# Unrepentant-Atheist/AC-3-ACM-Codec

Hardware: AMD Instinct MI355X
Metric: AC-3 5.1@48kHz frames/sec/GPU (decode+encode); achieved HBM GB/s vs peak (higher is better)
Workload: dtype f32+i32

## Files before the change

### ac-3-acm-codec_amd/csrc/enc_syntax.h

```cpp
#pragma once
#include <stdint.h>

#ifndef __HIPCC__
#ifndef __host__
#define __host__
#endif
#ifndef __device__
#define __device__
#endif
#endif

namespace ac3mi {

#define SYN_FN __host__ __device__ inline __attribute__((always_inline))

constexpr int sdecaycod = 2, fdecaycod = 1, sgaincod = 1, dbkneecod = 2, floorcod = 4, fgaincod = 4;
constexpr int CPL_FLEAK = 0, CPL_SLEAK = 0;
constexpr int SYN_CPL = -1;

template <class D>
struct SynWriter {
    uint32_t pos = 0;
    uint64_t acc = 0;
    int nacc = 0;
    SYN_FN void put(int n, uint32_t v) { acc = (acc << n) | v; nacc += n; }
    SYN_FN void flush()
    {
        if (nacc > 32) {
            static_cast<D *>(this)->store(pos, nacc - 32, (uint32_t)(acc >> 32) & (0xffffffffu >> (64 - nacc)));
            pos += nacc - 32;
            nacc = 32;
        }
        if (nacc > 0) {
            static_cast<D *>(this)->store(pos, nacc, (uint32_t)acc & (0xffffffffu >> (32 - nacc)));
            pos += nacc;
            nacc = 0;
        }
    }
};

struct SynCounter {
    int bits = 0;
    SYN_FN void put(int n, uint32_t) { bits += n; }
    SYN_FN void flush() {}
    SYN_FN void exponents(int, int, int ng) { bits += 4 + 7 * ng; }
};

template <class K>
SYN_FN void syn_header(K &k, uint32_t fscod, uint32_t frmsizecod, uint32_t bsid, int acmod, bool lfe, bool dual, uint32_t m,
                       uint32_t compr0, uint32_t compr1)
{
    k.put(16, 0x0b77); k.put(16, 0); k.put(2, fscod); k.put(6, frmsizecod); k.put(5, bsid); k.put(3, (m >> 5) & 7u); k.put(3, (uint32_t)acmod);
    k.flush();
    if ((acmod & 1) && acmod != 1) k.put(2, (m >> 8) & 3u);
    if (acmod & 4) k.put(2, (m >> 10) & 3u);
    if (acmod == 2) k.put(2, (m >> 12) & 3u);
    k.put(1, lfe);
    auto programme = [&](uint32_t c) {
        k.put(5, m & 31u);
        if (c & 0x100u) { k.put(1, 1); k.put(8, c & 0xffu); } else k.put(1, 0);
        k.put(2, 0);
    };
    programme(compr0);
    if (dual) programme(compr1);
    k.put(1, (m >> 14) & 1u); k.put(1, (m >> 15) & 1u); k.put(3, 0);
    k.flush();
}

struct SynShape {
    int acmod, nfbw, nch;
    bool lfe, dual;
    int nbc;
    uint32_t chbwcod;
};
struct SynCpl {
    uint32_t word;
    int begf, endf;
    uint32_t strat;
};

SYN_FN int syn_grpsize(int strat) { return strat == 1 ? 1 : strat == 2 ? 2 : 4; }
SYN_FN int syn_exp_groups(int n, int strat)
{
    const int gs = syn_grpsize(strat);
    return (n + gs * 3 - 4) / (3 * gs);
}
SYN_FN int syn_cpl_exp_groups(int cs, int ce, int strat) { return (ce - cs) / (3 * syn_grpsize(strat)); }
SYN_FN int syn_cpl_nrem(int begf) { return begf == 0 ? 2 : begf <= 2 ? 3 : 4; }

template <class K, class Blksw, class Dynrng, class Strat, class Cplco>
SYN_FN void syn_block(K &k, const SynShape &s, const SynCpl &c, int b, Blksw blksw, Dynrng dynrng, uint32_t remat, Strat strat_of,
                      Cplco cplco, uint32_t csnr, uint32_t fsnr)
{
    const int nfbw = s.nfbw, nch = s.nch;
    const bool cplf = (c.word & 1u) != 0;
    const int cs = 37 + 12 * c.begf, ce = 73 + 12 * c.endf, ncb = 3 + c.endf - c.begf;
    for (int ch = 0; ch < nfbw; ch++) k.put(1, blksw(ch));
    for (int ch = 0; ch < nfbw; ch++) k.put(1, 1);
    auto dynrng_word = [&](uint32_t w) {
        if (w & 0x100u) { k.put(1, 1); k.put(8, w & 0xffu); k.flush(); }
        else k.put(1, 0);
    };
    dynrng_word(dynrng(0));
    if (s.dual) dynrng_word(dynrng(1));
    if (cplf) {
        if (b == 0) {
            k.put(1, 1); k.put(1, 1);
            for (int ch = 0; ch < nfbw; ch++) k.put(1, 1);
            if (s.acmod == 2) k.put(1, 0);
            k.put(4, (uint32_t)c.begf); k.put(4, (uint32_t)c.endf); k.put(ncb - 1, 0);
            k.flush();
            for (int ch = 0; ch < nfbw; ch++) {
                k.put(1, 1); k.put(2, (c.word >> (8 + 2 * ch)) & 3u);
                for (int bd = 0; bd < ncb; bd++) { k.put(8, cplco(ch, bd)); if ((bd & 3) == 3) k.flush(); }
                k.flush();
            }
        } else {
            k.put(1, 0);
            for (int ch = 0; ch < nfbw; ch++) k.put(1, 0);
        }
    } else if (b == 0) { k.put(1, 1); k.put(1, 0); } else k.put(1, 0);
    if (s.acmod == 2) {
        const int nrem = cplf ? syn_cpl_nrem(c.begf) : 4;
        k.put(1, remat >> 4);
        if (remat & 0x10u) for (int i = 0; i < nrem; i++) k.put(1, (remat >> i) & 1u);
    }
    if (cplf) k.put(2, c.strat);
    for (int ch = 0; ch < nfbw; ch++) k.put(2, strat_of(ch));
    if (s.lfe) k.put(1, strat_of(nch - 1));
    for (int ch = 0; ch < nfbw; ch++) if (strat_of(ch) != 0 && !cplf) k.put(6, s.chbwcod);
    if (cplf && c.strat != 0) k.exponents(SYN_CPL, (int)c.strat, syn_cpl_exp_groups(cs, ce, (int)c.strat));
    for (int ch = 0; ch < nch; ch++) {
        const int stg = (int)strat_of(ch);
        if (stg == 0) continue;
        const bool is_lfe = s.lfe && ch == nch - 1;
        k.exponents(ch, stg, syn_exp_groups(is_lfe ? 7 : cplf ? cs : s.nbc, stg));
        if (!is_lfe) k.put(2, 0);
    }
    if (b == 0) k.flush();
    k.put(1, b == 0);
    if (b == 0) { k.put(2, sdecaycod); k.put(2, fdecaycod); k.put(2, sgaincod); k.put(2, dbkneecod); k.put(3, floorcod); }
    k.put(1, b == 0);
    if (b == 0) {
        k.put(6, csnr);
        if (cplf) { k.put(4, fsnr); k.put(3, fgaincod); k.flush(); }
        for (int ch = 0; ch < nch; ch++) { k.put(4, fsnr); k.put(3, fgaincod); }
    }
    if (cplf) {
        k.put(1, b == 0);
        if (b == 0) { k.put(3, CPL_FLEAK); k.put(3, CPL_SLEAK); }
    }
    k.put(1, 0);
    k.put(1, 0);
    k.flush();
}

SYN_FN int syn_header_bits(int acmod, uint32_t compr0, uint32_t compr1)
{
    return 16 + 16 + 2 + 6 + 5 + 3 + 3 + (((acmod & 1) && acmod != 1) ? 2 : 0) + ((acmod & 4) ? 2 : 0) + (acmod == 2 ? 2 : 0) + 1 + 5 + 3 +
           (acmod == 0 ? 8 : 0) + 1 + 1 + 3 + ((compr0 & 0x100u) ? 8 : 0) + ((compr1 & 0x100u) ? 8 : 0);
}
template <class Strat>
SYN_FN int syn_block_bits(const SynShape &s, int b, uint32_t dynrng0, uint32_t dynrng1, uint32_t remat, Strat strat_of)
{
    const int nfbw = s.nfbw, nch = s.nch;
    int bits = 2 * nfbw + 1 + (s.dual ? 1 : 0) + (b == 0 ? 2 : 1) + (s.acmod == 2 ? 1 + ((remat & 0x10u) ? 4 : 0) : 0) + 2 * nfbw + (s.lfe ? 1 : 0) +
               1 + (b == 0 ? 11 : 0) + 1 + (b == 0 ? 6 + 7 * nch : 0) + 2;
    bits += ((dynrng0 & 0x100u) ? 8 : 0) + ((dynrng1 & 0x100u) ? 8 : 0);
    for (int ch = 0; ch < nch; ch++) {
        const int stg = (int)strat_of(ch);
        if (stg == 0) continue;
        const bool is_lfe = s.lfe && ch == nch - 1;
        bits += 4 + 7 * syn_exp_groups(is_lfe ? 7 : s.nbc, stg) + (is_lfe ? 0 : 8);
    }
    return bits;
}

SYN_FN int syn_priced_fixed(int acmod, bool lfe, int nfbw, int nch)
{
    const int extra[8] = {8, 0, 2, 2, 2, 4, 2, 4};
    int bits = 65 + extra[acmod & 7];
    bits += 6 * (nfbw * 2 + 2 + (acmod == 2 ? 1 : 0) + (acmod == 0 ? 1 : 0) + 2 * nfbw + (lfe ? 1 : 0) + 1 + 1 + 2);
    bits++;
    bits += 2 * 4 + 3 + 6 + nch * (4 + 3);
    bits += 2;
    bits += 16;
    return bits;
}
SYN_FN int syn_priced_cpl(int acmod, int nfbw, int nb)
{
    return nfbw + (acmod == 2 ? 1 : 0) + 8 + (nb - 1) + nfbw * (3 + 8 * nb) + 5 * nfbw + 6 * 2 + 7 + 7 + 5;
}
}
```

### ac-3-acm-codec_amd/csrc/encode.hip

```cpp
#include "ac3mi_internal.h"
#include "wave_ops.h"
#include "spec_tables.h"
#include "enc_mant.h"
#include "enc_syntax.h"
#include "enc_exp.h"
#include "snr_window.h"

#include <type_traits>

namespace ac3mi {

__device__ __forceinline__ int ilog2u(unsigned v) { return v ? 31 - __builtin_clz(v) : 0; }

__device__ __forceinline__ int wave_sum(int v) { return (int)wave_sum_u32((uint32_t)v); }


struct PackParams {
    const int32_t *mdct;
    const uint8_t *eexp;
    const int16_t *emask;
    const uint8_t *strat;
    const int32_t *ebits;
    const int8_t *shift;
    int32_t *csnr_state;
    const int32_t *slot;
    int32_t *snr;
    uint32_t *memo;
    uint8_t *frames;
    const EncTables *tab;
    uint8_t *tap_eexp;
    uint8_t *tap_bap;
    uint8_t *tap_strat;
    int32_t *tap_snr;
    int32_t *tap_curve;
    int n_streams, frames_per_stream, frame_stride;
    int nch, nfbw, lfe, acmod, fscod, halfrate, bsid, frmsizecod, frame_words;
    int nbc;
    int chbwcod;
    uint16_t crc_inv_t[16];
    uint16_t pw1_t[6][16], pw2_t[6][16];
    int c1, c2;
    int frw;
    int marker;
    const uint32_t *hint;
    int hint_stride;
    const uint8_t *bsw;
    const uint8_t *remat;
    CplWs cpl;
    int cpl_begf;
    int cpl_endf;
    const uint8_t *drc;
    uint32_t bsi;
    const uint32_t *bsi_words;
    const uint8_t *dyn;
    const uint16_t *compr;
};

__device__ __forceinline__ uint32_t pack_bsi(const PackParams &P, size_t fidx)
{
    return P.bsi_words ? bsi_sanitise((uint32_t)__builtin_amdgcn_readfirstlane((int)P.bsi_words[fidx])) : P.bsi;
}

__device__ __forceinline__ bool drc_sends(const uint8_t *code, int b) { return b == 0 || code[b] != code[b - 1]; }
__device__ __forceinline__ bool dyn_sends(const uint8_t *code, int b, int p) { return code[2 * b + p] != (b ? code[2 * b - 2 + p] : 0); }
__device__ __forceinline__ uint32_t compr_word(const PackParams &P, size_t fidx, int p)
{
    return P.compr ? (uint32_t)__builtin_amdgcn_readfirstlane((int)P.compr[fidx * 2 + p]) & 0x1ffu : 0u;
}

template <bool MD, bool DW>
__device__ __forceinline__ uint32_t pack_dynrng(const PackParams &P, size_t fidx, int b, int p)
{
    if constexpr (DW) if (P.dyn) return dyn_sends(P.dyn + fidx * 12, b, p) ? 0x100u | P.dyn[fidx * 12 + 2 * b + p] : 0u;
    if constexpr (MD) if (P.drc && drc_sends(P.drc + fidx * 6, b)) return 0x100u | P.drc[fidx * 6 + b];
    return 0u;
}

struct MaskTabs {
    uint8_t latab[256];
    uint16_t hth[50];
    uint8_t band_of_bin[256];
    uint8_t band_start[52];
};

template <bool CPL>
struct SearchMaskRows {
    int16_t mask[CPL ? 42 : 36][50];
};
struct SearchWindowBufs {
    alignas(16) uint32_t scan[4 + 256];
    alignas(16) uint32_t hist[4][6][15][2];
};
template <bool CPL, bool WIN>
struct alignas(16) SearchLDS : std::conditional_t<WIN, SearchWindowBufs, SearchMaskRows<CPL>> {
    uint32_t bitlut[64];
    uint8_t strat[6][6];
    uint8_t band_of_bin[256];
    uint32_t rowdesc[CPL ? 42 : 36];
    uint2 terms[2][50];
};

__device__ __forceinline__ void put_bits(uint32_t *fr, int frw, uint32_t pos, int n, uint32_t v)
{
    if (n <= 0) return;
    const uint32_t w = pos >> 5;
    if (w + 1 >= (uint32_t)frw) return;
    const uint64_t x = (uint64_t)v << (64 - n - (pos & 31));
    const uint32_t hi = (uint32_t)(x >> 32), lo = (uint32_t)x;
    if (hi) atomicOr(&fr[w], hi);
    if (lo) atomicOr(&fr[w + 1], lo);
}

__device__ __forceinline__ uint32_t pick_row(const uint32_t (&ew)[6], int row, uint32_t other)
{
    uint32_t dw = other;
#pragma unroll
    for (int c2 = 0; c2 < 6; c2++) dw = c2 == row ? ew[c2] : dw;
    return dw;
}

template <class Row>
struct PackSink : SynWriter<PackSink<Row>> {
    uint32_t *fr;
    int frw, lane;
    uint8_t *erow;
    Row row_of;
    int cs;
    __device__ __forceinline__ PackSink(uint32_t *fr_, int frw_, int lane_, uint8_t *erow_, Row row_of_, int cs_, uint32_t at)
        : fr(fr_), frw(frw_), lane(lane_), erow(erow_), row_of(row_of_), cs(cs_) { this->pos = at; }
    __device__ __forceinline__ void store(uint32_t at, int n, uint32_t v) { if (lane == 0) put_bits(fr, frw, at, n, v); }
    __device__ __forceinline__ void exponents(int row, int strat, int ng)
    {
        const int gs = syn_grpsize(strat), first = row == SYN_CPL ? cs : 1;
        const uint8_t *e = erow;
        const uint32_t dw = row_of(row);
        wave_sync();
        *reinterpret_cast<uint32_t *>(&erow[4 * lane]) = dw;
        wave_sync();
        this->put(4, (uint32_t)__builtin_amdgcn_readfirstlane((int)e[first - 1]) >> (row == SYN_CPL ? 1 : 0));
        this->flush();
        for (int g = lane; g < ng; g += 64) {
            const int k0 = first + 3 * g * gs;
            const int prev = g ? e[k0 - gs] : e[first - 1];
            const int d0 = e[k0] - prev + 2, d1 = e[k0 + gs] - e[k0] + 2, d2 = e[k0 + 2 * gs] - e[k0 + gs] + 2;
            put_bits(fr, frw, this->pos + 7 * g, 7, (uint32_t)((d0 * 5 + d1) * 5 + d2));
        }
        this->pos += 7 * ng;
    }
};


__device__ __forceinline__ uint32_t bytes_min_where(uint32_t a, uint32_t b, uint32_t where)
{
    const uint32_t ge = (((a | 0x80808080u) - b) >> 7) & 0x01010101u;
    const uint32_t m = ((ge << 8) - ge) & where;
    return (b & m) | (a & ~m);
}

template <int PER>
__device__ __forceinline__ int encode_exp_wave_t(uint8_t *row, int n, int lane)
{
    const int groups = syn_exp_groups(n, exp_strategy_of<PER>), ng = 3 * groups;
    uint32_t *q = reinterpret_cast<uint32_t *>(row);
    const uint32_t own = q[lane], nxt = q[lane + 1];
    int bin[4], g[PER], ix[PER];
    bool valid[PER];
    const int row0 = chan_exp_entries<PER>(own, nxt, ng, lane, bin, g, ix, valid);
    const int head = exp_constrain<PER, true>(g, ix, valid, row0, lane);
    const int row0new = head < row0 ? head : row0;
    uint32_t o = 0;
#pragma unroll
    for (int k = 0; k < 4; k++) o |= (uint32_t)(valid[k * PER / 4] ? g[k * PER / 4] : bin[k]) << (8 * k);
    const uint32_t prev = (uint32_t)__builtin_amdgcn_update_dpp(row0new << 24, (int)o, 0x138, 0xf, 0xf, false);
    q[lane] = __builtin_amdgcn_alignbyte(o, prev, 3u);
    return 4 + 7 * groups;
}

__device__ int encode_exp_wave(uint8_t *row, int n, int strategy, int lane)
{
    if (strategy == 1) return encode_exp_wave_t<4>(row, n, lane);
    if (strategy == 2) return encode_exp_wave_t<2>(row, n, lane);
    return encode_exp_wave_t<1>(row, n, lane);
}

template <int PER>
__device__ __forceinline__ int encode_exp_sum_t(uint32_t own, int n, int lane)
{
    constexpr int gs = 4 / PER;
    const int ng = 3 * syn_exp_groups(n, exp_strategy_of<PER>);
    const uint32_t nxt = (uint32_t)__builtin_amdgcn_update_dpp(0, (int)own, 0x130, 0xf, 0xf, false);
    int bin[4], g[PER], ix[PER];
    bool valid[PER];
    const int row0 = chan_exp_entries<PER>(own, nxt, ng, lane, bin, g, ix, valid);
    const int head = exp_constrain<PER, true>(g, ix, valid, row0, lane);
    int sum = lane == 0 ? (head < row0 ? head : row0) : 0;
#pragma unroll
    for (int c = 0; c < PER; c++) {
        int cnt = n - (4 * lane + 1 + c * gs);
        cnt = cnt < 0 ? 0 : cnt > gs ? gs : cnt;
        sum += valid[c] ? g[c] * cnt : 0;
    }
    return sum;
}

__device__ __forceinline__ int cpl_exp_sum(const uint8_t *row, int cs, int ce, int strategy, int lane)
{
    const int gs = syn_grpsize(strategy);
    int g[3], ix[3];
    bool valid[3];
    cpl_exp_entries(row, cs, 3 * syn_cpl_exp_groups(cs, ce, strategy), gs, lane, g, ix, valid);
    exp_constrain<3, false>(g, ix, valid, 0, lane);
    int sum = 0;
#pragma unroll
    for (int c = 0; c < 3; c++) sum += valid[c] ? g[c] * gs : 0;
    return sum;
}

template <bool CPLROW>
__device__ uint32_t xs_choose(const uint8_t (*E)[256], uint8_t *scratch, uint32_t in, int n, int cs, int ce, int extra,
                              bool d15, int lane)
{
    int bits[3];
#pragma unroll
    for (int s = 0; s < 3; s++) bits[s] = 4 + 7 * (CPLROW ? syn_cpl_exp_groups(cs, ce, s + 1) : syn_exp_groups(n, s + 1)) + extra;
    int J1 = 0, J2 = 0, J3 = 0, J4 = 0, J5 = 0, J6 = 0;
    uint32_t choice = 0;
#pragma unroll 1
    for (int i = 5; i >= 0; i--) {
        uint32_t acc = *reinterpret_cast<const uint32_t *>(&E[i][4 * lane]);
        uint32_t racc = 0;
        int best = 0x7fffffff, bl = 1, bs = 1;
#pragma unroll 1
        for (int L = 1; L <= 6 - i; L++) {
            const uint32_t rb = *reinterpret_cast<const uint32_t *>(&E[i + L - 1][4 * lane]);
            if (L > 1) acc = bytes_min_where(acc, rb, in);
            racc = __builtin_amdgcn_sad_u8(rb & in, 0u, racc);
            int c15, c25 = 0, c45 = 0;
            if constexpr (CPLROW) {
                *reinterpret_cast<uint32_t *>(&scratch[4 * lane]) = acc;
                wave_sync();
                c15 = cpl_exp_sum(scratch, cs, ce, 1, lane);
                c25 = cpl_exp_sum(scratch, cs, ce, 2, lane);
                c45 = cpl_exp_sum(scratch, cs, ce, 3, lane);
                wave_sync();
            } else {
                c15 = encode_exp_sum_t<4>(acc, n, lane);
                if (!d15) {
                    c25 = encode_exp_sum_t<2>(acc, n, lane);
                    c45 = encode_exp_sum_t<1>(acc, n, lane);
                }
            }
            const uint32_t a = wave_sum_u32((uint32_t)c15 | (uint32_t)c25 << 16);
            const uint32_t b = wave_sum_u32((uint32_t)c45 | racc << 16);
            const int R = (int)(b >> 16);
            const int k = i + L;
            const int Jn = k == 1 ? J1 : k == 2 ? J2 : k == 3 ? J3 : k == 4 ? J4 : k == 5 ? J5 : J6;
            const int C[3] = {(int)(a & 0xffffu), (int)(a >> 16), (int)(b & 0xffffu)};
#pragma unroll
            for (int s = 0; s < 3; s++) {
                if (s > 0 && d15) break;
                const int cost = bits[s] + R - L * C[s] + Jn;
                if (cost < best) { best = cost; bl = L; bs = s + 1; }
            }
        }
        J1 = i == 1 ? best : J1; J2 = i == 2 ? best : J2; J3 = i == 3 ? best : J3;
        J4 = i == 4 ? best : J4; J5 = i == 5 ? best : J5;
        choice |= (uint32_t)(bl | bs << 3) << (5 * i);
    }
    uint32_t st = 0;
    for (int i = 0; i < 6;) {
        const int c = (int)((choice >> (5 * i)) & 31u);
        st |= (uint32_t)(c >> 3) << (4 * i);
        i += c & 7;
    }
    return st;
}

__device__ __forceinline__ void mask_leaks(int psd, bool live, int b, int sdecay, int fdecay, int sgain, int fgain, int &fast, int &slow)
{
    constexpr int NEG = -0x3fffffff;
    fast = live ? psd - fgain + b * fdecay : NEG;
    slow = live ? psd - sgain + b * sdecay : NEG;
    wave_incl_scan_max2(fast, slow);
    fast -= b * fdecay;
    slow -= b * sdecay;
}
__device__ __forceinline__ void mask_store(const MaskTabs &T, int16_t *mask, int b, bool inside, int excite, int psd, int dbknee, int halfrate)
{
    const int t = dbknee - psd;
    if (t > 0) excite += t >> 2;
    const int h = T.hth[(b < 50 ? b : 49) >> halfrate];
    if (b < 50) mask[b] = inside ? (int16_t)(excite > h ? excite : h) : (int16_t)0;
}

__device__ void mask_row_wave(const MaskTabs &T, int16_t *bndpsd, int bndend, bool is_lfe, int sdecay, int fdecay, int sgain,
                              int dbknee, int fgain, int halfrate, int lane)
{
    constexpr int NEG = -0x3fffffff;
    const int b = lane;
    const int cur = b < bndend ? bndpsd[b] : 0;
    const int nxt = (b + 1 < bndend && !(is_lfe && b == 6)) ? bndpsd[b + 1] : 0;
    const bool skip = (is_lfe && b == 6) || b >= 22 || b >= bndend;
    const bool reset = !skip && b < 20 && cur + 256 == nxt;
// ... 1438 lines not shown
                win_slope15 = __builtin_amdgcn_readlane(spare, 0) - __builtin_amdgcn_readlane(spare, 15);
                win_cmin = lo < win_cmin ? lo : win_cmin;
                win_cmax = lo + 15 > win_cmax ? lo + 15 : win_cmax;
                if constexpr (!FX) if (P.tap_curve && lane < WIN_N) {
                    P.tap_curve[(fidx * 1024 + lo + lane) * 2] = spare;
                    P.tap_curve[(fidx * 1024 + lo + lane) * 2 + 1] = extra6;
                }
            }
          }
        };
        bool first_sweep = true;
        const bool cold_hint = csnr_prev == 40 && fsnr_prev == 0;
        if constexpr (WIN) {
            for (;;) {
                int cc, ff;
                bool more;
                while ((more = ss.next(cc, ff))) {
                    bool fits;
                    if (!lookup(cc, ff, fits)) break;
                    ss.consume(fits);
                }
                if (!more) break;
                int lo;
                if (win_sweeps == 0) {
                    const int hint0 = (cold_hint && P.hint) ? (int)__builtin_amdgcn_readfirstlane((int)P.hint[fidx * (size_t)P.hint_stride]) : 0;
                    lo = win_first_lo(hint0, cold_hint, 16 * csnr_prev + fsnr_prev);
                } else {
                    lo = win_next_lo(win_sweeps, gl, spare_l, gh, spare_h, win_slope15, win_cmin, win_cmax, 16 * cc + ff);
                }
                win_sweeps++;
                cost_window(lo);
            }
        } else
        for (;;) {
            int cc, ff;
            bool more;
            while ((more = ss.next(cc, ff))) {
                bool fits;
                if (!lookup(cc, ff, fits)) break;
                if (ss.phase == 0 && !fits) went_down = true;
                if (ss.phase == 1 && fits) went_up = true;
                ss.consume(fits);
            }
            if (!more) break;
            int cg[ENC_NC], n_cand = 0;
#pragma unroll
            for (int k = 0; k < ENC_NC; k++) cg[k] = -1;
            auto add = [&](int g) {
                bool dup = false;
#pragma unroll
                for (int k = 0; k < ENC_NC; k++) dup = dup || cg[k] == g;
                if (dup) return false;
#pragma unroll
                for (int k = 0; k < ENC_NC; k++) cg[k] = k == n_cand ? g : cg[k];
                n_cand++;
                return true;
            };
            bool probing = false;
            if (probe_sweeps < 3 && gl >= 0 && gh > gl + 3) {
                const int w = gh - gl;
                const float est = (float)w * ((float)spare_l / (float)(spare_l - spare_h));
                int d = w > 48 ? (w * 85) >> 10 : 1;
                d = d < 2 && w > 48 ? 2 : d;
                const int ge = gl + (int)(est + 0.5f);
                auto clampg = [&](int g) { return g < gl + 1 ? gl + 1 : g > gh - 1 ? gh - 1 : g; };
                add(clampg(ge));
                add(clampg(ge + d));
                add(clampg(ge - d));
                for (int k = 1; n_cand < ENC_NC && k < w; k++) {
                    if (ge - k > gl && ge - k < gh) add(ge - k);
                    if (n_cand < ENC_NC && ge + k > gl && ge + k < gh) add(ge + k);
                }
                probe_sweeps++;
                probing = true;
            }
            const int hint0 = (first_sweep && cold_hint && P.hint) ? (int)__builtin_amdgcn_readfirstlane((int)P.hint[fidx * (size_t)P.hint_stride]) : 0;
            if (n_cand == 0 && hint0 > 0) {
                const int g0 = hint0 < 8 ? 8 : hint0 > 1000 ? 1000 : hint0;
                add(g0 - 8); add(g0 + 2); add(g0 + 12);
            }
            if (n_cand == 0 && first_sweep && cold_hint) {
                add(16 * 8); add(16 * 13); add(16 * 20);
            }
            if (n_cand == 0 && ss.phase == 0 && (went_down || (first_sweep && cold_hint))) {
                int n = 0;
                for (int c = ss.csnr; c >= 0 && n < 16; c -= 4, n++) { bool f; if (lookup(c, 0, f)) break; }
                if (n > 3) {
                    add(16 * (ss.csnr - 4 * ((n - 1) / 4)));
                    add(16 * (ss.csnr - 4 * ((n - 1) / 2)));
                    add(16 * (ss.csnr - 4 * ((3 * (n - 1) + 2) / 4)));
                }
            }
            first_sweep = false;
            if (n_cand == 0) {
                SnrSearch ahead = ss;
                while (n_cand < ENC_NC && ahead.next(cc, ff)) {
                    bool fits;
                    if (!lookup(cc, ff, fits)) {
                        if (!add(16 * cc + ff)) break;
                        fits = ahead.phase == 0 ? !went_down : ahead.phase == 1 ? went_up : true;
                    }
                    ahead.consume(fits);
                }
            }
            cost_and_record(cg, n_cand, probing);
        }
        if (PART == 3) {
            const int C = ss.failed ? 0 : ss.csnr;
            for (;;) {
                int cg[ENC_NC], n_cand = 0;
#pragma unroll
                for (int k = 0; k < ENC_NC; k++) cg[k] = -1;
                for (int c = C - 7 < 0 ? 0 : C - 7; c <= (C + 8 > 63 ? 63 : C + 8) && n_cand < ENC_NC; c++) {
                    if ((known_c >> c) & 1) continue;
#pragma unroll
                    for (int k = 0; k < ENC_NC; k++) cg[k] = k == n_cand ? 16 * c : cg[k];
                    n_cand++;
                }
                if (n_cand == 0) break;
                cost_and_record(cg, n_cand, false);
            }
            if (lane == 0) {
                uint32_t *m = P.memo + fidx * 8;
                m[0] = (uint32_t)known_c; m[1] = (uint32_t)(known_c >> 32);
                m[2] = (uint32_t)fits_c; m[3] = (uint32_t)(fits_c >> 32);
                m[4] = known_f; m[5] = fits_f; m[6] = (uint32_t)f_cc; m[7] = 0;
            }
            continue;
        }
        int csnr = ss.csnr, fsnr = ss.fsnr;
        int failed_alloc = -1;
        {
            if (!ss.failed) { csnr_prev = csnr; fsnr_prev = fsnr; }
            else {
                failed_alloc = csnr_prev & 3;
                csnr = csnr_prev;
                fsnr = fsnr_prev;
            }
        }
        if (!FX && P.tap_snr && lane == 0) { P.tap_snr[fidx * 2] = csnr; P.tap_snr[fidx * 2 + 1] = fsnr; }
        if (!FX && P.tap_strat && lane < 36) {
            const int b = lane / 6, ch = lane - 6 * b;
            if (ch < nch) P.tap_strat[(fidx * 6 + b) * nch + ch] = L.strat[b][ch];
        }
        if (lane == 0) { P.snr[fidx * 2] = csnr; P.snr[fidx * 2 + 1] = fsnr | (failed_alloc >= 0 ? 0x100 | (failed_alloc << 9) : 0); }
        PK_LAP(0);
    }
    if (PART == 1 && lane == 0) P.csnr_state[sslot] = csnr_prev | (fsnr_prev << 8);
    PK_END();
}



template <bool CPL>
struct alignas(16) PackfLDS {
    int16_t mask[CPL ? 7 : 6][50];
    uint4 packlut[64];
    alignas(16) uint16_t glist[GL_ENTRIES];
    alignas(4) uint8_t erow[256];
    alignas(4) uint16_t crc_tab[256];
};

#ifndef ENC_PACK2_LB
#define ENC_PACK2_LB 4
#endif
template <bool FIXED51, bool CPL = false, bool BW = false, bool MD = false, bool DUAL = false, bool DW = false>
__global__ __launch_bounds__(64, ENC_PACK2_LB) void enc_packf_kernel(const PackParams P)
{
    static_assert(!DW || MD, "the array words are written where the profiles' are");
    static_assert(!(FIXED51 && CPL), "coupled frames take the generic packer");
    static_assert(!(DUAL && (FIXED51 || CPL)), "dual mono is neither 5.1 nor coupled");
    __shared__ PackfLDS<CPL> L;
    extern __shared__ uint4 pk_dyn[];
    uint32_t *fr = reinterpret_cast<uint32_t *>(pk_dyn);
    const int lane = threadIdx.x;
    PK_DECL();

    for (int i = lane; i < 256; i += 64) L.crc_tab[i] = P.tab->crc_tab[i];
    {
        const int bp = P.tab->baptab[lane];
        L.packlut[lane] = mant_pack_entry(bp, plain_bits(bp));
    }
    mant_lists_init(L.glist, lane);
    const uint32_t bandoff = *reinterpret_cast<const uint32_t *>(&P.tab->band_of_bin[4 * lane]);
    const int nch = FIXED51 ? 6 : P.nch, nfbw = FIXED51 ? 5 : P.nfbw, nbc = FIXED51 && !BW ? 223 : P.nbc;
    const int acmod = FIXED51 ? 7 : P.acmod;
    const bool lfe = FIXED51 ? true : P.lfe != 0;
    const int fs = P.frame_words;
    const size_t fidx = blockIdx.x;
    const uint32_t cplw = CPL ? (uint32_t)__builtin_amdgcn_readfirstlane((int)P.cpl.word[fidx]) : 0u;
    const bool cplf = (cplw & 1u) != 0;
    const int cs = 37 + 12 * P.cpl_begf;
    const int cendf = BW ? P.cpl_endf : 12, ce = 73 + 12 * cendf;
    PK_T0();
    PK_COUNT(7);
    for (int i = lane; i < P.frw / 4; i += 64) reinterpret_cast<uint4 *>(fr)[i] = make_uint4(0, 0, 0, 0);
    const int32_t *md = P.mdct + fidx * 6 * nch * 256;
    const uint8_t *ex = P.eexp + fidx * 6 * nch * 256;
    int strat_l = 0, shift_l = 0;
    if (lane < 36) {
        const int b = lane / 6, ch = lane - 6 * b;
        if (ch < nch) { strat_l = (int)P.strat[(fidx * 6 + b) * nch + ch]; shift_l = (int)P.shift[(fidx * 6 + b) * nch + ch]; }
    }
    int csnr, fsnr, snroffset;
    {
        const int w1 = __builtin_amdgcn_readfirstlane(P.snr[fidx * 2 + 1]);
        csnr = __builtin_amdgcn_readfirstlane(P.snr[fidx * 2]);
        fsnr = w1 & 15;
        snroffset = (((csnr - 15) << 4) + fsnr) << 2;
        if (w1 & 0x100) snroffset = (((w1 >> 9) - 15) << 4) << 2;
    }
    wave_sync();
    PK_LAP(6);

    uint32_t pos;
    {
        PackSink k(fr, P.frw, lane, L.erow, [](int) { return 0u; }, cs, 0u);
        syn_header(k, P.fscod, P.frmsizecod, P.bsid, acmod, lfe, DUAL, MD ? pack_bsi(P, fidx) : BSI_DEFAULT,
                   DW ? compr_word(P, fidx, 0) : 0u, DW && DUAL ? compr_word(P, fidx, 1) : 0u);
        pos = k.pos;
    }
    const SynShape shape{acmod, nfbw, nch, lfe, DUAL, nbc, (uint32_t)P.chbwcod};

#pragma unroll 1
    for (int b = 0; b < 6; b++) {
        uint32_t ew[6];
#pragma unroll
        for (int ch = 0; ch < 6; ch++) ew[ch] = ch < nch ? *reinterpret_cast<const uint32_t *>(ex + ((size_t)b * nch + ch) * 256 + 4 * lane) : 0u;
        uint32_t cew = 0;
        int cstg = 0;
        if (cplf) {
            cew = *reinterpret_cast<const uint32_t *>(P.cpl.eexp + (fidx * 6 + b) * 256 + 4 * lane);
            cstg = __builtin_amdgcn_readfirstlane((int)P.cpl.strat[fidx * 8 + b]);
            if (lane < 25)
                reinterpret_cast<uint32_t *>(&L.mask[CPL ? 6 : 0][0])[lane] =
                    mant_band_terms(reinterpret_cast<const uint32_t *>(P.cpl.emask + (fidx * 6 + b) * 50)[lane], snroffset);
        }
        {
            const uint32_t *gm = reinterpret_cast<const uint32_t *>(P.emask + (fidx * 6 + b) * nch * 50);
            uint32_t mv[3];
#pragma unroll
            for (int j = 0; j < 3; j++) mv[j] = lane + 64 * j < nch * 25 ? gm[lane + 64 * j] : 0u;
#pragma unroll
            for (int j = 0; j < 3; j++)
                if (lane + 64 * j < nch * 25) reinterpret_cast<uint32_t *>(&L.mask[0][0])[lane + 64 * j] = mant_band_terms(mv[j], snroffset);
        }
        auto strat_of = [&](int ch) { return (uint32_t)__builtin_amdgcn_readlane(strat_l, 6 * b + ch); };
        const uint8_t *bs = P.bsw ? P.bsw + (fidx * 6 + b) * nch : nullptr;
        PackSink k(fr, P.frw, lane, L.erow, [&](int row) { return pick_row(ew, row, cew); }, cs, pos);
        syn_block(k, shape, SynCpl{cplw, P.cpl_begf, cendf, (uint32_t)cstg}, b,
                  [&](int ch) -> uint32_t { return bs ? bs[ch] : 0u; },
                  [&](int p) { return pack_dynrng<MD, DW>(P, fidx, b, p); },
                  acmod == 2 && P.remat ? (uint32_t)P.remat[fidx * 6 + b] : b == 0 ? 0x10u : 0u, strat_of,
                  [&](int ch, int bd) -> uint32_t { return P.cpl.co[fidx * 80 + ch * 16 + bd]; }, (uint32_t)csnr, (uint32_t)fsnr);
        pos = k.pos;
        PK_LAP(1);

        {
            int shv[6];
#pragma unroll
            for (int ch = 0; ch < 6; ch++) shv[ch] = __builtin_amdgcn_readlane(shift_l, 6 * b + ch);
            if (CPL && cplf) {
                MantBlock B;
                B.fr = fr; B.frw = P.frw; B.glist = L.glist; B.packlut = L.packlut;
                B.mdb = md + (size_t)b * nch * 256;
                B.tap_bap = P.tap_bap ? P.tap_bap + (fidx * 6 + b) * nch * 256 : nullptr;
                B.nch = nch; B.nbc = nbc; B.lfe = lfe; B.marker = (uint32_t)P.marker;
                const int csh = __builtin_amdgcn_readfirstlane((int)P.cpl.shift[fidx * 8 + b]);
                auto beyond = [&](int n) { const int k = n - 4 * lane; return k >= 4 ? 0u : k <= 0 ? 0xffffffffu : 0xffffffffu << (8 * k); };
                const uint32_t um_cch = beyond(cs), um_cpl = ~beyond(cs) | beyond(ce), um_lfe = beyond(7);
                uint32_t ad7[7], em7[7];
                int sh7[7], neg = 0;
#pragma unroll
                for (int p = 0; p < 7; p++) {
                    const int c = p == 0 ? 0 : p == 6 ? nch - 1 : p - 1;
                    const bool on = p == 1 || (p == 6 ? lfe : p == 0 || p - 1 < nfbw);
                    uint32_t e = 0;
                    int sv = 0, trow = 0;
#pragma unroll
                    for (int c2 = 0; c2 < 6; c2++) { e = c2 == c ? ew[c2] : e; sv = c2 == c ? shv[c2] : sv; }
                    trow = c;
                    if (p == 1) { e = cew; sv = csh; trow = 6; }
                    ad7[p] = 0; em7[p] = 0; sh7[p] = sv;
                    if (on) {
                        em7[p] = e | (p == 1 ? um_cpl : p == 6 ? um_lfe : um_cch);
#pragma unroll
                        for (int j = 0; j < 4; j++) {
                            const int xe = (int)((em7[p] >> (8 * j)) & 0xff);
                            int a = (int)L.mask[trow][(bandoff >> (8 * j)) & 0xff] - 4 * xe;
                            a = a < 0 ? 0 : a > 63 ? 63 : a;
                            ad7[p] |= (uint32_t)a << (8 * j);
                            neg |= xe - sv;
                        }
                    }
                }
                PK_LAP(8);
                B.cplrow = P.cpl.mdct + (fidx * 6 + b) * 256;
                pos = mant_pack_block<true>(B, em7, ad7, sh7, __ballot(neg < 0) != 0, pos, lane);
            } else {
                uint32_t ad[6];
                int neg;
                uint32_t em[6];
                mant_block_addresses(ad, em, neg, ew, shv, L.mask, bandoff, nch, nbc, lfe, lane);
                PK_LAP(8);
                MantBlock B;
                B.fr = fr; B.frw = P.frw; B.glist = L.glist; B.packlut = L.packlut;
                B.mdb = md + (size_t)b * nch * 256;
                B.tap_bap = P.tap_bap ? P.tap_bap + (fidx * 6 + b) * nch * 256 : nullptr;
                B.nch = nch; B.nbc = nbc; B.lfe = lfe; B.marker = (uint32_t)P.marker;
                pos = mant_pack_block(B, em, ad, shv, __ballot(neg < 0) != 0, pos, lane);
            }
        }
        PK_LAP(2);
    }

    const int fs58 = (fs >> 1) + (fs >> 3);
    uint32_t crc1 = region_crc(L, fr, 2 * fs58, 2 * fs58, P.c1, P.pw1_t, 4, lane);
    crc1 = gf_mul_tab(crc1, P.crc_inv_t);
    const uint32_t crc2 = region_crc(L, fr, 2 * fs - 2, (fs - fs58) * 2 - 2, P.c2, P.pw2_t, 0, lane);
    wave_sync();
    if (lane == 0) {
        fr[0] = (fr[0] & 0xffff0000u) | (crc1 & 0xffff);
        const int p = 2 * fs - 2;
        const int shft = 16 - 8 * (p & 3);
        fr[p >> 2] = (fr[p >> 2] & ~(0xffffu << shft)) | ((crc2 & 0xffff) << shft);
    }
    wave_sync();
    uint8_t *dst = P.frames + fidx * P.frame_stride;
    for (int i = lane; i < (2 * fs + 3) / 4; i += 64) {
        uint32_t v = __builtin_bswap32(fr[i]);
        const int rem = 2 * fs - 4 * i;
        if (rem >= 4) *reinterpret_cast<uint32_t *>(dst + 4 * i) = v;
        else for (int k = 0; k < rem; k++) dst[4 * i + k] = (uint8_t)(v >> (8 * k));
    }
    PK_LAP(3);
    PK_END();
}


struct PackbWave {
    int16_t mask[6][50];
    alignas(16) uint16_t glist[GL_ENTRIES];
    alignas(4) uint8_t erow[256];
};
struct alignas(16) PackbLDS {
    PackbWave w[6];
    uint4 packlut[64];
    uint16_t crc_tab[256];
    uint8_t band_of_bin[256];
    uint32_t blk_bits[6];
    uint32_t blk_bits2[6];
    uint32_t crc[2];
    int any_coll;
};

#ifndef ENC_PACKB_LB
#define ENC_PACKB_LB 4
#endif
template <bool MD = false, bool DW = false>
__global__ __launch_bounds__(384, ENC_PACKB_LB) void enc_packb_kernel(const PackParams P)
{
    static_assert(!DW || MD, "the array words are written where the profiles' are");
    __shared__ PackbLDS L;
    extern __shared__ uint4 pk_dyn[];
    uint32_t *fr = reinterpret_cast<uint32_t *>(pk_dyn);
    const int tid = threadIdx.x, lane = tid & 63;
    const int b = __builtin_amdgcn_readfirstlane(tid >> 6);
    PackbWave &W = L.w[b];
    const size_t fidx = xcd_remap(blockIdx.x, gridDim.x);
    const int nch = P.nch, nfbw = P.nfbw, nbc = P.nbc, fs = P.frame_words;

    for (int i = tid; i < 256; i += 384) {
        L.band_of_bin[i] = P.tab->band_of_bin[i];
        L.crc_tab[i] = P.tab->crc_tab[i];
    }
    if (tid < 64) { const int bp = P.tab->baptab[tid]; L.packlut[tid] = mant_pack_entry(bp, plain_bits(bp)); }
    for (int i = tid; i < P.frw / 4; i += 384) reinterpret_cast<uint4 *>(fr)[i] = make_uint4(0, 0, 0, 0);
    const size_t rowb = (fidx * 6 + b) * nch;
    uint32_t mrows[3] = {0u, 0u, 0u};
    {
        const uint32_t *gm = reinterpret_cast<const uint32_t *>(P.emask + rowb * 50);
#pragma unroll
        for (int j = 0; j < 3; j++)
            if (lane + 64 * j < nch * 25) mrows[j] = gm[lane + 64 * j];
    }
    const int strat_l = lane < nch ? (int)P.strat[rowb + lane] : 0;
    const int shift_l = lane < nch ? (int)P.shift[rowb + lane] : 0;
    uint32_t ew[6];
#pragma unroll
    for (int ch = 0; ch < 6; ch++) ew[ch] = ch < nch ? *reinterpret_cast<const uint32_t *>(P.eexp + (rowb + ch) * 256 + 4 * lane) : 0u;
    int csnr, fsnr, snroffset;
    {
        const int w1 = P.snr[fidx * 2 + 1];
        csnr = P.snr[fidx * 2];
        fsnr = w1 & 15;
        snroffset = (((csnr - 15) << 4) + fsnr) << 2;
        if (w1 & 0x100) snroffset = (((w1 >> 9) - 15) << 4) << 2;
    }
    if (tid == 0) L.any_coll = 0;
    mant_lists_init(W.glist, lane);
#pragma unroll
    for (int j = 0; j < 3; j++)
        if (lane + 64 * j < nch * 25) reinterpret_cast<uint32_t *>(&W.mask[0][0])[lane + 64 * j] = mant_band_terms(mrows[j], snroffset);
    const uint32_t bandoff = *reinterpret_cast<const uint32_t *>(&P.tab->band_of_bin[4 * lane]);
    __syncthreads();

    const uint32_t strat_lo = (uint32_t)__ballot(strat_l & 1), strat_hi = (uint32_t)__ballot(strat_l & 2);
    auto strat_of = [&](int ch) { return ((strat_lo >> ch) & 1u) | (((strat_hi >> ch) & 1u) << 1); };
// ... 510 lines not shown
```

Before: 9.615 million.

## Precompute 5.1 block syntax bit images and write them with parallel ORs

```diff
diff --git a/ac-3-acm-codec_amd/csrc/enc_syntax.h b/ac-3-acm-codec_amd/csrc/enc_syntax.h
--- a/ac-3-acm-codec_amd/csrc/enc_syntax.h
+++ b/ac-3-acm-codec_amd/csrc/enc_syntax.h
@@ -176,6 +176,66 @@
     return bits;
 }
 
+struct SynImages51 {
+    uint32_t pre[2], suf[2];
+    int pre_bits, suf_bits, suf_at, bits;
+    int absexp_at[6], gainrng_at[6];
+};
+template <class Strat>
+SYN_FN void syn_block_images_51(SynImages51 &im, int b, uint32_t blksw, Strat strat_of, int nbc, uint32_t chbwcod, uint32_t csnr, uint32_t fsnr)
+{
+    uint64_t acc = ((uint64_t)blksw << 5) | 31u;
+    acc = b == 0 ? (acc << 3) | 2u : acc << 2;
+    int n = b == 0 ? 13 : 12;
+    for (int ch = 0; ch < 5; ch++) acc = (acc << 2) | strat_of(ch);
+    acc = (acc << 1) | strat_of(5);
+    n += 11;
+    for (int ch = 0; ch < 5; ch++)
+        if (strat_of(ch) != 0) { acc = (acc << 6) | chbwcod; n += 6; }
+    im.pre_bits = n;
+    acc <<= 64 - n;
+    im.pre[0] = (uint32_t)(acc >> 32);
+    im.pre[1] = (uint32_t)acc;
+    int at = n;
+    for (int ch = 0; ch < 6; ch++) {
+        const int stg = (int)strat_of(ch);
+        im.absexp_at[ch] = im.gainrng_at[ch] = 0;
+        if (stg == 0) continue;
+        im.absexp_at[ch] = at;
+        at += 4 + 7 * syn_exp_groups(ch == 5 ? 7 : nbc, stg);
+        if (ch < 5) { im.gainrng_at[ch] = at; at += 2; }
+    }
+    im.suf_at = at;
+    uint64_t s = (1u << 11) | (sdecaycod << 9) | (fdecaycod << 7) | (sgaincod << 5) | (dbkneecod << 3) | floorcod;
+    s = (((s << 1) | 1u) << 6) | csnr;
+    for (int ch = 0; ch < 6; ch++) s = (((s << 4) | fsnr) << 3) | fgaincod;
+    s <<= 3;
+    im.suf[0] = b == 0 ? (uint32_t)(s >> 32) : 0u;
+    im.suf[1] = b == 0 ? (uint32_t)s : 0u;
+    im.suf_bits = b == 0 ? 63 : 4;
+    im.bits = at + im.suf_bits;
+}
+SYN_FN uint32_t syn_image_dword(uint32_t w0, uint32_t w1, int j, uint32_t at)
+{
+    const uint32_t a = j == 1 ? w0 : j == 2 ? w1 : 0u, c = j == 0 ? w0 : j == 1 ? w1 : 0u, s = at & 31u;
+    return s ? (a << (32u - s)) | (c >> s) : c;
+}
+constexpr int SYN_HEADER_BITS_51 = 69;
+SYN_FN void syn_header_image_51(uint32_t (&w)[3], uint32_t fscod, uint32_t frmsizecod, uint32_t bsid, uint32_t m)
+{
+    w[0] = 0x0b770000u;
+    uint32_t v = (fscod << 6) | frmsizecod;
+    v = (v << 5) | bsid;
+    v = (v << 3) | ((m >> 5) & 7u);
+    v = (v << 3) | 7u;
+    v = (v << 2) | ((m >> 8) & 3u);
+    v = (v << 2) | ((m >> 10) & 3u);
+    v = (v << 1) | 1u;
+    v = (v << 5) | (m & 31u);
+    w[1] = v << 3;
+    w[2] = ((((m >> 14) & 1u) << 1) | ((m >> 15) & 1u)) << 30;
+}
+
 SYN_FN int syn_priced_fixed(int acmod, bool lfe, int nfbw, int nch)
 {
     const int extra[8] = {8, 0, 2, 2, 2, 4, 2, 4};
diff --git a/ac-3-acm-codec_amd/csrc/encode.hip b/ac-3-acm-codec_amd/csrc/encode.hip
--- a/ac-3-acm-codec_amd/csrc/encode.hip
+++ b/ac-3-acm-codec_amd/csrc/encode.hip
@@ -149,6 +149,29 @@
     }
 };
 
+__device__ __forceinline__ void or_image(uint32_t *fr, int frw, const uint32_t *w, uint32_t at, int lane)
+{
+    if (lane < 3) {
+        const uint32_t d = syn_image_dword(w[0], w[1], lane, at), i = (at >> 5) + (uint32_t)lane;
+        if (d && i + 1 < (uint32_t)frw) atomicOr(&fr[i], d);
+    }
+}
+__device__ __forceinline__ void exp_row_at(uint32_t *fr, int frw, uint8_t *erow, uint32_t dw, uint32_t at, int strat, int ng, int lane)
+{
+    const int gs = syn_grpsize(strat);
+    const uint8_t *e = erow;
+    wave_sync();
+    *reinterpret_cast<uint32_t *>(&erow[4 * lane]) = dw;
+    wave_sync();
+    for (int g = lane; g < ng; g += 64) {
+        const int k0 = 1 + 3 * g * gs;
+        const int prev = g ? e[k0 - gs] : e[0];
+        const int d0 = e[k0] - prev + 2, d1 = e[k0 + gs] - e[k0] + 2, d2 = e[k0 + 2 * gs] - e[k0 + gs] + 2;
+        const uint32_t code = (uint32_t)((d0 * 5 + d1) * 5 + d2);
+        put_bits(fr, frw, g ? at + 4 + 7 * g : at, g ? 7 : 11, g ? code : ((uint32_t)e[0] << 7) | code);
+    }
+}
+
 
 __device__ __forceinline__ uint32_t bytes_min_where(uint32_t a, uint32_t b, uint32_t where)
 {
@@ -1893,8 +1916,14 @@
 
 
 
-template <bool CPL>
-struct alignas(16) PackfLDS {
+struct PackfImages {
+    alignas(16) uint16_t at[6][8];
+    uint32_t pre[6][2];
+    uint32_t suf0[2];
+};
+struct PackfNoImages {};
+template <bool CPL, bool IMG = false>
+struct alignas(16) PackfLDS : std::conditional_t<IMG, PackfImages, PackfNoImages> {
     int16_t mask[CPL ? 7 : 6][50];
     uint4 packlut[64];
     alignas(16) uint16_t glist[GL_ENTRIES];
@@ -1911,7 +1940,8 @@
     static_assert(!DW || MD, "the array words are written where the profiles' are");
     static_assert(!(FIXED51 && CPL), "coupled frames take the generic packer");
     static_assert(!(DUAL && (FIXED51 || CPL)), "dual mono is neither 5.1 nor coupled");
-    __shared__ PackfLDS<CPL> L;
+    constexpr bool IMG = FIXED51 && !CPL && !MD && !DUAL && !DW;
+    __shared__ PackfLDS<CPL, IMG> L;
     extern __shared__ uint4 pk_dyn[];
     uint32_t *fr = reinterpret_cast<uint32_t *>(pk_dyn);
     const int lane = threadIdx.x;
@@ -1951,11 +1981,34 @@
         snroffset = (((csnr - 15) << 4) + fsnr) << 2;
         if (w1 & 0x100) snroffset = (((w1 >> 9) - 15) << 4) << 2;
     }
+    if constexpr (IMG) {
+        const uint64_t s_lo = __ballot(strat_l & 1), s_hi = __ballot(strat_l & 2);
+        if (lane < 6) {
+            const uint32_t lo = (uint32_t)(s_lo >> (6 * lane)) & 63u, hi = (uint32_t)(s_hi >> (6 * lane)) & 63u;
+            uint32_t bswm = 0;
+            if (P.bsw) {
+#pragma unroll
+                for (int ch = 0; ch < 5; ch++) bswm = (bswm << 1) | P.bsw[(fidx * 6 + lane) * 6 + ch];
+            }
+            SynImages51 im;
+            syn_block_images_51(im, lane, bswm, [&](int ch) { return ((lo >> ch) & 1u) | (((hi >> ch) & 1u) << 1); }, nbc, (uint32_t)P.chbwcod,
+                                (uint32_t)csnr, (uint32_t)fsnr);
+            *reinterpret_cast<uint4 *>(L.at[lane]) = make_uint4((uint32_t)(im.absexp_at[0] | im.absexp_at[1] << 16), (uint32_t)(im.absexp_at[2] | im.absexp_at[3] << 16),
+                                                                (uint32_t)(im.absexp_at[4] | im.absexp_at[5] << 16), (uint32_t)(im.suf_at | im.bits << 16));
+            *reinterpret_cast<uint2 *>(L.pre[lane]) = make_uint2(im.pre[0], im.pre[1]);
+            if (lane == 0) *reinterpret_cast<uint2 *>(L.suf0) = make_uint2(im.suf[0], im.suf[1]);
+        }
+    }
     wave_sync();
     PK_LAP(6);
 
     uint32_t pos;
-    {
+    if constexpr (IMG) {
+        uint32_t hw[3];
+        syn_header_image_51(hw, (uint32_t)P.fscod, (uint32_t)P.frmsizecod, (uint32_t)P.bsid, BSI_DEFAULT);
+        if (lane < 3) fr[lane] = lane == 0 ? hw[0] : lane == 1 ? hw[1] : hw[2];
+        pos = SYN_HEADER_BITS_51;
+    } else {
         PackSink k(fr, P.frw, lane, L.erow, [](int) { return 0u; }, cs, 0u);
         syn_header(k, P.fscod, P.frmsizecod, P.bsid, acmod, lfe, DUAL, MD ? pack_bsi(P, fidx) : BSI_DEFAULT,
                    DW ? compr_word(P, fidx, 0) : 0u, DW && DUAL ? compr_word(P, fidx, 1) : 0u);
@@ -1987,14 +2040,28 @@
                 if (lane + 64 * j < nch * 25) reinterpret_cast<uint32_t *>(&L.mask[0][0])[lane + 64 * j] = mant_band_terms(mv[j], snroffset);
         }
         auto strat_of = [&](int ch) { return (uint32_t)__builtin_amdgcn_readlane(strat_l, 6 * b + ch); };
-        const uint8_t *bs = P.bsw ? P.bsw + (fidx * 6 + b) * nch : nullptr;
-        PackSink k(fr, P.frw, lane, L.erow, [&](int row) { return pick_row(ew, row, cew); }, cs, pos);
-        syn_block(k, shape, SynCpl{cplw, P.cpl_begf, cendf, (uint32_t)cstg}, b,
-                  [&](int ch) -> uint32_t { return bs ? bs[ch] : 0u; },
-                  [&](int p) { return pack_dynrng<MD, DW>(P, fidx, b, p); },
-                  acmod == 2 && P.remat ? (uint32_t)P.remat[fidx * 6 + b] : b == 0 ? 0x10u : 0u, strat_of,
-                  [&](int ch, int bd) -> uint32_t { return P.cpl.co[fidx * 80 + ch * 16 + bd]; }, (uint32_t)csnr, (uint32_t)fsnr);
-        pos = k.pos;
+        if constexpr (IMG) {
+            const uint4 atw = *reinterpret_cast<const uint4 *>(L.at[b]);
+            or_image(fr, P.frw, L.pre[b], pos, lane);
+#pragma unroll
+            for (int ch = 0; ch < 6; ch++) {
+                const int stg = (int)strat_of(ch);
+                if (stg == 0) continue;
+                const uint32_t pair = ch < 2 ? atw.x : ch < 4 ? atw.y : atw.z;
+                exp_row_at(fr, P.frw, L.erow, ew[ch], pos + ((ch & 1) ? pair >> 16 : pair & 0xffffu), stg, syn_exp_groups(ch == 5 ? 7 : nbc, stg), lane);
+            }
+            if (b == 0) or_image(fr, P.frw, L.suf0, pos + (atw.w & 0xffffu), lane);
+            pos += (uint32_t)__builtin_amdgcn_readfirstlane((int)(atw.w >> 16));
+        } else {
+            const uint8_t *bs = P.bsw ? P.bsw + (fidx * 6 + b) * nch : nullptr;
+            PackSink k(fr, P.frw, lane, L.erow, [&](int row) { return pick_row(ew, row, cew); }, cs, pos);
+            syn_block(k, shape, SynCpl{cplw, P.cpl_begf, cendf, (uint32_t)cstg}, b,
+                      [&](int ch) -> uint32_t { return bs ? bs[ch] : 0u; },
+                      [&](int p) { return pack_dynrng<MD, DW>(P, fidx, b, p); },
+                      acmod == 2 && P.remat ? (uint32_t)P.remat[fidx * 6 + b] : b == 0 ? 0x10u : 0u, strat_of,
+                      [&](int ch, int bd) -> uint32_t { return P.cpl.co[fidx * 80 + ch * 16 + bd]; }, (uint32_t)csnr, (uint32_t)fsnr);
+            pos = k.pos;
+        }
         PK_LAP(1);
 
         {
```

New measurement: 9.722 million (median of 6 runs). 1.1% higher.
